# tmaklin/kbo

Measured on AMD Instinct MI355X. Metric: query Mbp/sec for kbo map, k=31, 5 Mbp SBWT; bit-exact MS vs CPU, higher is better.
Workload: dtype u32

## Files before the change

kbo_amd/batch.py:

```python
import ctypes as C

import numpy as np

from . import _capi, derandomize
from ._capi import check, lib


def _prep(concat, offsets):
    concat = np.ascontiguousarray(concat, dtype=np.uint8)
    offsets = np.ascontiguousarray(offsets, dtype=np.uint64)
    return concat, offsets, len(offsets) - 1


def ms_batch(sbwt, concat, offsets, want_intervals=False):
    concat, offsets, n = _prep(concat, offsets)
    total = int(offsets[-1]) if n > 0 else 0
    d = np.zeros(max(total, 1), dtype=np.uint8)
    lo = np.zeros(max(total, 1), dtype=np.uint32) if want_intervals else None
    hi = np.zeros(max(total, 1), dtype=np.uint32) if want_intervals else None
    check(lib().kbo_ms_batch(sbwt._h, concat.ctypes.data, offsets.ctypes.data, n, d.ctypes.data,
                             lo.ctypes.data if want_intervals else None,
                             hi.ctypes.data if want_intervals else None))
    return d[:total], (lo[:total] if want_intervals else None), (hi[:total] if want_intervals else None)

# ... 398 lines not shown
            self.work = torch.zeros(self.work_bytes // 8 + 2, dtype=torch.int64, device=device)
            self.lo = torch.zeros(self.total, dtype=torch.int32, device=device) if want_intervals else None
            self.hi = torch.zeros(self.total, dtype=torch.int32, device=device) if want_intervals else None
        self.format = format
        self.want_ms = want_ms
        self.max_error_prob = max_error_prob
        self.fused = None

    def walk(self, stream=None):
        s = stream if stream is not None else self.torch.cuda.current_stream(self.device)
        check(lib().kbo_ms_batch_dev(self.sbwt._h, self.q.data_ptr(), self.off.data_ptr(), self.n_seqs,
                                     self.total, self.max_len, self.ms.data_ptr(),
                                     self.lo.data_ptr() if self.lo is not None else None,
                                     self.hi.data_ptr() if self.hi is not None else None,
                                     self.work.data_ptr(), self.work_bytes, s.cuda_stream))

    def plan_stats(self, stream=None):
        s = stream if stream is not None else self.torch.cuda.current_stream(self.device)
        out = np.zeros(20, dtype=np.uint64)
        check(lib().kbo_plan_stats_dev(self.n_seqs, self.total, self.max_len, self.k, self.work.data_ptr(), out.ctypes.data,
                                       s.cuda_stream))
        names = ("units_walked", "accepted", "failed", "levels", "entry_levels", "seed_lookups", "seed_extensions",
                 "mismatches", "units", "redo_entries", "gave_up", "guard", "tab_lookups", "tab_written", "tab_flagged",
                 "tab_unresolved", "tab_anchored", "items_noplan")
        return {n: int(v) for n, v in zip(names, out)}

    def plan_flags(self, stream=None):
        s = stream if stream is not None else self.torch.cuda.current_stream(self.device)
        out = np.zeros(self.n_seqs, dtype=np.uint8)
        check(lib().kbo_plan_flags_dev(self.n_seqs, self.total, self.max_len, self.k, self.work.data_ptr(), out.ctypes.data, s.cuda_stream))
        return out

    def long_stats(self, stream=None):
        s = stream if stream is not None else self.torch.cuda.current_stream(self.device)
        out = np.zeros(25, dtype=np.uint64)
        check(lib().kbo_long_stats_dev(self.n_seqs, self.total, self.max_len, self.k, self.work.data_ptr(), out.ctypes.data, s.cuda_stream))
        names = ("pieces", "flagged", "sub_items", "seed_lookups", "filter_lookups", "table_lookups", "second_lookups", "_",
                 "cyc_staging", "cyc_stretches", "cyc_planes", "cyc_proof", "cyc_output", "band_tried", "band_taken", "_",
                 "why_other", "why_list", "why_ext", "why_back", "why_on", "why_band_list", "why_band_ext", "why_band_back", "why_band_on")
        return {n: int(v) for n, v in zip(names, out) if n != "_"}

    def derand_translate(self, stream=None):
        s = stream if stream is not None else self.torch.cuda.current_stream(self.device)
        if self.max_len == 0 or self.max_len > 480:
            if getattr(self, "dt_work", None) is None:
                self.dt_work_bytes = int(lib().kbo_derand_work_bytes(self.n_seqs, self.total))
                self.dt_work = self.torch.zeros(self.dt_work_bytes // 8 + 2, dtype=self.torch.int64, device=self.device)
# ... 228 lines not shown
```

kbo_amd/csrc/capi_internal.hpp:

```cpp
#pragma once
#include <atomic>
#include <cstdint>
#include <map>
#include <memory>
#include <mutex>
#include <string>
#include <vector>

#include "host_util.hpp"
#include "kernels.hpp"
#include "refine.hpp"
#include "sbwt_index.hpp"

namespace kbo_host {

struct DevCopy {
    bool arena_borrowed = false;
    static bool &transient_arena_in_use()
    {
        static thread_local bool in_use = false;
        return in_use;
    }
    DevBuf arena;
    DevBuf ent;
    uint64_t n_blocks = 0;
    bool big = false;
    uint32_t pair_off = 0;
    DevBuf seed_tab;
    uint32_t seed_d = 0;
    DevBuf dtab;
    uint32_t dtab_order = 0;
    bool dtab_grouped = false;
    DevBuf anchor;
    uint32_t anchor_bits = 0;
    DevBuf fat;
    uint32_t fat_null = 0;
    DevBuf pc_text, pc_pos, pc_node;
    DevBuf dfilt;
    uint32_t dfilt_bases = 0;
    DevBuf pc_tm, seed_pos;
    DevBuf pc_t, pc_mu, pc_mc;
    bool plan_built = false;
    bool plan_failed = false;
    uint64_t bases_seen = 0;
    struct Setup {
        double layout_s = 0, cover_s = 0, lines_s = 0, seed_s = 0, dtab_s = 0, upload_s = 0;
        uint64_t rank_bytes = 0, entry_bytes = 0, pair_bytes = 0, cover_bytes = 0, lines_bytes = 0, seed_bytes = 0, dtab_bytes = 0,
                 anchor_bytes = 0;
    } setup;
    struct PlanState {
        std::atomic<int> holdoff{0};
        std::atomic<uint32_t> epoch{0};
        uint32_t *bailed = nullptr;
        std::atomic<uint32_t> bails{0};
    } plan;
    ~DevCopy()
    {
        if (plan.bailed) {
            int prev = -1;
            (void)hipGetDevice(&prev);
            if (arena.dev >= 0 && arena.dev != prev) (void)hipSetDevice(arena.dev);
            (void)hipDeviceSynchronize();
            if (arena.dev >= 0 && arena.dev != prev && prev >= 0) (void)hipSetDevice(prev);
            (void)hipHostFree(plan.bailed);
// ... 364 lines not shown
```

kbo_amd/csrc/device_batch.cpp:

```cpp
#include "../../include/kbo_hip.h"
#include "../../include/kbo_hip_tuning.h"

#include <hip/hip_runtime.h>

#include <algorithm>
#include <atomic>
#include <cstdlib>
#include <deque>
#include <memory>
#include <mutex>
#include <vector>

#include "batch_route.hpp"

using namespace kbo_host;


namespace {
struct DevWork {
    bool chunked;
    uint32_t chunk, n_slots;
    size_t scan_off, plan_off, ms_bytes, bytes;
    size_t long_off, long_bytes, derand_off, derand_bytes;
    size_t shard_off, shard_bytes;
// ... 150 lines not shown
}

int kbo_plan_stats_dev(size_t n_seqs, uint64_t total_bases, size_t max_seq_len, uint32_t k, const void *d_work,
                       uint64_t out[KBO_PLAN_STATS], void *stream)
{
    return guarded([&] {
        KBO_REQUIRE(d_work && out && n_seqs > 0 && total_bases > 0, KBO_E_BAD_ARG, "null / empty argument");
        const DevWork w = dev_work(n_seqs, total_bases, max_seq_len, k, false);
        const kbo::PlanLayout L = kbo::plan_layout(w.n_slots, total_bases);
        const uint8_t *plan = static_cast<const uint8_t *>(d_work) + w.plan_off;
        hipStream_t s = static_cast<hipStream_t>(stream);
        uint32_t ctl[16], st[kbo::kPlanStatSlots * kbo::kPlanStatWords], tot[2];
        const uint32_t last = 2u * w.n_slots;
        HIP_OK(hipMemcpyAsync(ctl, plan + L.qctl, sizeof ctl, hipMemcpyDeviceToHost, s));
        HIP_OK(hipMemcpyAsync(st, plan + L.pstats, sizeof st, hipMemcpyDeviceToHost, s));
        HIP_OK(hipMemcpyAsync(&tot[0], plan + L.ucount + (size_t)last * 4, 4, hipMemcpyDeviceToHost, s));
        HIP_OK(hipMemcpyAsync(&tot[1], plan + L.usums + (size_t)(last / 1024u) * 4, 4, hipMemcpyDeviceToHost, s));
        HIP_OK(hipStreamSynchronize(s));
        for (uint32_t i = 0; i < KBO_PLAN_STATS; i++) out[i] = 0;
        for (uint32_t sl = 0; sl < kbo::kPlanStatSlots; sl++) {
            for (uint32_t i = 0; i < 8; i++) out[i] += st[sl * kbo::kPlanStatWords + i];
            for (uint32_t i = 0; i < 3; i++) out[12 + i] += st[sl * kbo::kPlanStatWords + kbo::kPlanStatTabLookups + i];
            out[16] += st[sl * kbo::kPlanStatWords + kbo::kPlanStatTabAnchored];
        }
        out[15] = ctl[4];
        out[17] = ctl[5];
        out[8] = (uint64_t)tot[0] + tot[1];
        out[9] = ctl[1];
        out[10] = ctl[2];
        out[11] = ctl[3];
    });
}

int kbo_plan_flags_dev(size_t n_seqs, uint64_t total_bases, size_t max_seq_len, uint32_t k, const void *d_work, uint8_t *flags_out, void *stream)
{
    return guarded([&] {
        KBO_REQUIRE(d_work && flags_out && n_seqs > 0 && total_bases > 0, KBO_E_BAD_ARG, "null / empty argument");
        const DevWork w = dev_work(n_seqs, total_bases, max_seq_len, k, false);
        KBO_REQUIRE(!w.chunked, KBO_E_UNSUPPORTED, "one item per sequence only (reads)");
        const kbo::PlanLayout L = kbo::plan_layout(w.n_slots, total_bases);
        hipStream_t s = static_cast<hipStream_t>(stream);
        HIP_OK(hipMemcpyAsync(flags_out, static_cast<const uint8_t *>(d_work) + w.plan_off + L.redo, n_seqs, hipMemcpyDeviceToHost, s));
        HIP_OK(hipStreamSynchronize(s));
    });
}

// ... 840 lines not shown
```

kbo_amd/csrc/device_index.cpp:

```cpp
#include "capi_internal.hpp"
#include "map_text.hpp"

#include <cmath>

#include <atomic>
#include <chrono>
#include <cstdlib>

namespace kbo_host {

std::atomic<int> g_waves_per_cu{0};
std::atomic<bool> g_force_big{false};
std::atomic<uint64_t> g_pair_min_rows{24ull << 20};
std::atomic<bool> g_plan_enabled{true};
std::atomic<int> g_plan_cap_div{1};
std::atomic<int> g_seed_table_depth{0};
std::atomic<int> g_depth_table{0};
std::atomic<int> g_depth_table_anchors{-1};

bool plan_enabled(const kbo_index *idx)
{
    const int v = idx ? idx->opts.plan.load() : kOptInherit;
    return v == kOptInherit ? g_plan_enabled.load() : v != 0;
}
// ... 234 lines not shown
        dc->setup.dtab_bytes = kbo::dtab_bytes((uint32_t)order, grouped) + (dc->dfilt_bases ? ((uint64_t)1 << (2u * dc->dfilt_bases)) / 8u : 0u);
        dc->setup.anchor_bytes = dc->anchor_bits ? ((uint64_t)1 << dc->anchor_bits) * 8 : 0;
    }
    dc->setup.seed_bytes = dc->seed_d ? (uint64_t)8 << (2u * dc->seed_d) : 0;
    if (dc->dtab_order >= 4 && dc->seed_d >= 4) {
        t0 = clk::now();
        const uint64_t units = kbo::pack_text_units(idx->host.n_sets);
        dc->pc_tm.alloc(units * 8 + 64);
        const uint64_t mu_bytes = kbo::pack_text_mu_bytes(units);
        dc->pc_t.alloc(units * 4 + 64);
        dc->pc_mu.alloc(mu_bytes + 64);
        dc->pc_mc.alloc(kbo::maptext::kCells / 8u);
        HIP_OK(hipMemsetAsync(dc->pc_t.as<uint8_t>() + units * 4, 0, 64, bs));
        HIP_OK(hipMemsetAsync(dc->pc_mu.as<uint8_t>() + mu_bytes, 0xFF, 64, bs));
        HIP_OK(kbo::launch_pack_text(dc->pc_text.as<uint8_t>(), pc.text.size(), dc->pc_tm.as<uint2>(), dc->pc_t.as<uint32_t>(), dc->pc_mu.as<uint32_t>(), dc->pc_mc.as<uint32_t>(), units,
                                     bs));
        dc->seed_pos.alloc(((size_t)4 << (2u * dc->seed_d)) + 64);
        HIP_OK(kbo::launch_seed_pos(dc->seed_tab.as<uint2>(), dc->pc_pos.as<uint32_t>(), dc->seed_pos.as<uint32_t>(), dc->seed_d, bs));
        HIP_OK(hipStreamSynchronize(bs));
        dc->setup.cover_bytes += units * 12 + mu_bytes + kbo::maptext::kCells / 8u;
        dc->setup.seed_bytes += (uint64_t)4 << (2u * dc->seed_d);
        idx->plan_bytes += units * 12 + mu_bytes + kbo::maptext::kCells / 8u + ((size_t)4 << (2u * dc->seed_d));
        dc->setup.seed_s += since(t0);
    }
    dc->plan_built = true;
}

uint64_t plan_break_even_bases(const kbo_index *idx)
{
    const int64_t set = g_plan_lazy_bases.load();
    if (set >= 0) return (uint64_t)set;
    const double rows = (double)idx->host.n_sets;
    const double setup_s = rows * ((idx->cover ? 0.0 : 50e-9) + 15e-9);
    if (setup_s < 0.1) return 0;
    return (uint64_t)(setup_s / 7e-12);
}
}

namespace {
void layout_from_device_rows(const kbo_index *idx, const uint64_t *d_rows, const uint8_t *d_lcs, size_t n_words, uint64_t n_blocks,
                             uint4 *d_rank, uint8_t *d_ent, uint4 *d_pair)
{
    const uint64_t n_rows = idx->host.n_sets;
    DevBuf d_scr(kbo::device_layout_scratch_bytes(n_rows));
    const uint64_t *rows_dev[4];
    for (int c = 0; c < 4; c++) rows_dev[c] = d_rows + (size_t)c * n_words;
// ... 73 lines not shown
            dc->setup.rank_bytes = rank_bytes;
            dc->setup.entry_bytes = ent_bytes;
            dc->setup.pair_bytes = pair_bytes;
            dc->setup.upload_s = since(t0);
        } catch (...) {
            delete dc;
            if (prev != device) (void)hipSetDevice(prev);
            throw;
        }
        if (prev != device) HIP_OK(hipSetDevice(prev));
        it = idx->dev.emplace(device, dc).first;
    }
    DevCopy *dc = it->second;
    const bool plan_on = plan_enabled(idx);
    if (prepare && dc->plan_failed && !dc->plan_built) dc->plan_failed = false;
    if (!dc->plan_built && !dc->plan_failed && plan_on && !idx->transient) {
        dc->bases_seen += work_bases;
        if (prepare || dc->bases_seen >= plan_break_even_bases(idx)) {
            int prev = current_device();
            if (prev != device) HIP_OK(hipSetDevice(device));
            try {
                build_plan_structures(idx, dc);
            } catch (const KboError &e) {
                for (DevBuf *b : {&dc->pc_text, &dc->pc_pos, &dc->pc_node, &dc->fat, &dc->seed_tab, &dc->dtab, &dc->anchor, &dc->dfilt, &dc->pc_tm, &dc->pc_t, &dc->pc_mu, &dc->pc_mc, &dc->seed_pos})
                    b->release();
                dc->seed_d = dc->dtab_order = dc->anchor_bits = dc->dfilt_bases = 0;
                dc->dtab_grouped = false;
                dc->fat_null = 0;
                dc->plan_failed = true;
                (void)hipGetLastError();
                if (prev != device) (void)hipSetDevice(prev);
                if (prepare) throw;
                last_error() = std::string("plan structures not built (the copy walks plainly): ") + e.what();
            } catch (...) {
                if (prev != device) (void)hipSetDevice(prev);
                throw;
            }
            if (prev != device && !dc->plan_failed) HIP_OK(hipSetDevice(prev));
        }
    }
    if (plan) *plan = &dc->plan;
    kbo::DevIndexView v;
    v.arena = dc->arena.as<uint4>();
    v.n_blocks = (uint32_t)dc->n_blocks;
    v.lcs_off = (uint32_t)(dc->n_blocks * 4 + 1);
    v.pair_off = dc->pair_off;
    v.ent = dc->big ? dc->ent.as<uint8_t>() : nullptr;
    v.big = dc->big ? 1u : 0u;
    v.n = (uint32_t)idx->host.n_sets;
    v.k = idx->host.k;
    v.pc_text = (plan_on && dc->pc_text.p) ? dc->pc_text.as<uint8_t>() + kbo::kPlanPad : nullptr;
    v.pc_pos = dc->pc_pos.as<uint32_t>();
    v.seed_tab = dc->seed_d ? dc->seed_tab.as<uint2>() : nullptr;
    v.seed_d = dc->seed_d;
    const bool use_tab = dc->dtab_order != 0 && depth_table_setting(idx) >= 0;
    v.dtab = use_tab ? dc->dtab.as<uint8_t>() : nullptr;
    v.dtab_order = use_tab ? dc->dtab_order : 0u;
    v.dtab_grouped = dc->dtab_grouped ? 1u : 0u;
    v.anchor = (use_tab && dc->anchor_bits) ? dc->anchor.as<uint64_t>() : nullptr;
    v.anchor_bits = dc->anchor_bits;
    v.fat = dc->fat.p ? dc->fat.as<uint8_t>() : nullptr;
    v.fat_null = dc->fat_null;
    v.pc_node = dc->pc_node.as<uint32_t>();
    v.pc_tm = (use_tab && dc->pc_tm.p) ? dc->pc_tm.as<uint2>() : nullptr;
    v.pc_t = (v.pc_tm && dc->pc_t.p && dc->pc_mu.p && dc->pc_mc.p) ? dc->pc_t.as<uint32_t>() : nullptr;
    v.pc_mu = v.pc_t ? dc->pc_mu.as<uint8_t>() : nullptr;
    v.pc_mc = v.pc_t ? dc->pc_mc.as<uint32_t>() : nullptr;
    v.pc_mc_shift = kbo::maptext::cell_shift(kbo::pack_text_units(idx->host.n_sets));
    v.dfilt = (use_tab && dc->dfilt_bases) ? dc->dfilt.as<uint32_t>() : nullptr;
    v.dfilt_bases = v.dfilt ? dc->dfilt_bases : 0u;
    v.seed_pos = (use_tab && dc->seed_pos.p) ? dc->seed_pos.as<uint32_t>() : nullptr;
    for (int c = 0; c < 4; c++) v.C[c] = (uint32_t)idx->host.C[c];
    v.C[4] = v.n;
    return v;
}

namespace {
constexpr int kPlanHoldoff = 16;
std::atomic<uint32_t> g_plan_epoch{1};
}

void plan_reset_holdoff() { g_plan_epoch.fetch_add(1); }

void plan_after_launch(const kbo::WalkArgs &a, hipStream_t stream, DevCopy::PlanState *ps)
{
    if (!a.gitems || !a.qctl || !ps || !ps->bailed) return;
    (void)hipMemcpyAsync(ps->bailed, a.qctl + 2, 8, hipMemcpyDeviceToHost, stream);
}

void attach_plan(kbo::WalkArgs &a, void *plan_work, DevCopy::PlanState *ps)
{
    a.gitems = nullptr;
    a.glist = nullptr;
// ... 53 lines not shown
```

kbo_amd/csrc/kernels.hpp:

```cpp
#pragma once
#include <hip/hip_runtime.h>

#include <cstdint>

#include "refset_plan.hpp"

namespace kbo {

struct DevIndexView {
    const uint4 *arena;
    uint32_t n_blocks;
    uint32_t lcs_off;
    uint32_t pair_off;
    const uint8_t *ent;
    uint32_t big;
    uint32_t n;
    uint32_t k;
    const uint8_t *pc_text;
    const uint32_t *pc_pos;
    const uint32_t *pc_node;
    uint32_t C[5];
    const uint2 *seed_tab;
    uint32_t seed_d;
    const uint8_t *fat;
    uint32_t fat_null;
    const uint8_t *dtab;
    uint32_t dtab_order;
    uint32_t dtab_grouped;
    const uint64_t *anchor;
    uint32_t anchor_bits;
    const uint2 *pc_tm;
    const uint32_t *seed_pos;
    const uint32_t *pc_t;
    const uint8_t *pc_mu;
    const uint32_t *pc_mc;
    uint32_t pc_mc_shift;
    const uint32_t *dfilt;
    uint32_t dfilt_bases;
};

struct alignas(16) WalkItem {
    uint64_t start;
    uint32_t len;
    uint32_t warm;
};

constexpr uint32_t kPlanPad = 64;
constexpr uint32_t kPlanList = 12;
constexpr uint32_t kPlanListMax = 28;
constexpr uint32_t kPlanNone = 0xFF;
constexpr uint32_t kPlanInf = 0xFFFE;
struct alignas(16) GuidedItem {
    uint32_t start;
    uint32_t p0;
    uint16_t len;
    uint16_t j_conv;
    uint16_t mm0;
    uint8_t warm;
    uint8_t n_mm;
};
enum : uint32_t { kUnitHead = 1u, kUnitPlain = 2u, kUnitToEnd = 4u };
// ... 46 lines not shown
    uint32_t *call_counts;
    uint32_t call_cap;
    uint32_t call_thr;
    uint32_t table_mode;
    uint32_t table_fused;
    uint32_t redo_piece;
    uint32_t max_item_len;
    const uint32_t *n_items_dev;
    uint8_t *chars_out;
    uint32_t map_thr, map_fmt, map_want_ms;
    uint32_t *host_bailed;
    uint32_t *run_counts;
    const uint64_t *seq_off;
    uint32_t uniform_len;
    const uint32_t *qp;
    uint32_t qp_wps;
    const uint32_t *qp_data, *qp_sums;
    const uint8_t *qp_exc;
    uint32_t *packed_out;
    uint4 *summary_out;
};
enum : uint32_t { kPlanStatUnits = 0, kPlanStatAccepted, kPlanStatFailed, kPlanStatLevels, kPlanStatEntryLevels,
                  kPlanStatSeedLookups, kPlanStatSeedExtensions, kPlanStatMismatches,
                  kPlanStatTabLookups, kPlanStatTabWritten, kPlanStatTabFlagged, kPlanStatTabAnchored, kPlanStatWords };
constexpr uint32_t kPlanStatSlots = 8;
struct PlanLayout {
    size_t gitems, units, glist, ucount, usums, qctl, pstats, redo, end;
    uint32_t unit_cap;
};
inline size_t plan_unit_cap(size_t n_items, uint64_t total_bases) { return 3 * n_items + total_bases / 64 + 64; }
inline PlanLayout plan_layout(size_t n_items, uint64_t total_bases)
{
    PlanLayout L;
    size_t w = 0;
    L.gitems = w;
    w += n_items * sizeof(GuidedItem);
    L.unit_cap = (uint32_t)(plan_unit_cap(n_items, total_bases) < 0x7FFFFF00ull ? plan_unit_cap(n_items, total_bases) : 0x7FFFFF00ull);
    L.units = w;
    w += (size_t)L.unit_cap * sizeof(WalkUnit);
    L.glist = w;
    w += (n_items * kPlanListMax * 2 + 15) / 16 * 16;
    L.ucount = w;
    w += (2 * n_items + 1) * 4;
    L.usums = w;
    w += (n_items / 512 + 4) * 4;
    w = (w + 15) / 16 * 16;
    L.qctl = w;
    w += 64;
    L.pstats = w;
    w += kPlanStatSlots * kPlanStatWords * 4;
    L.redo = w;
    w += (n_items + 15) / 16 * 16;
    L.end = w;
    return L;
}
inline size_t plan_work_bytes(size_t n_items, uint64_t total_bases) { return plan_layout(n_items, total_bases).end + 64; }
hipError_t launch_plan(WalkArgs &a, hipStream_t stream);
hipError_t launch_ms_walk_guided(WalkArgs a, uint32_t grid, uint32_t threads, hipStream_t stream);
hipError_t launch_plan_table(WalkArgs &a, hipStream_t stream);
hipError_t launch_dtab_resolve(const WalkArgs &a, hipStream_t stream);
hipError_t launch_pack_text(const uint8_t *d_text_padded, uint64_t n_bytes, uint2 *d_out, uint32_t *d_t, uint32_t *d_mu, uint32_t *d_mc, uint64_t n_units,
                            hipStream_t stream);
constexpr uint32_t kMapPad = 192;
inline uint64_t pack_text_units(uint64_t n_sets) { return (n_sets + kMapPad + 256u) / 16u + 2u; }
inline uint64_t pack_text_mu_bytes(uint64_t n_units) { return (n_units + 255u) / 256u * 32u; }
hipError_t launch_seed_pos(const uint2 *d_seed_tab, const uint32_t *d_pc_pos, uint32_t *d_out, uint32_t seed_d, hipStream_t stream);
bool map_reads_applies(const WalkArgs &a);
hipError_t launch_map_reads(WalkArgs &a, hipStream_t stream);
bool map_reads_finish_applies(const WalkArgs &a);
hipError_t launch_map_reads_finish(const WalkArgs &a, hipStream_t stream, bool one_wave_groups = false);
bool map_reads_direct(const WalkArgs &a);
bool map_reads_summary_applies(const DevIndexView &ix, uint32_t longest);
bool map_reads_packed_applies(const WalkArgs &a, bool packed_out);
hipError_t launch_flag_exceptions(const uint64_t *d_pos, uint32_t n, uint64_t base, const uint64_t *d_off, uint32_t n_seqs, uint8_t *d_exc, hipStream_t stream);
hipError_t launch_unpack_flagged(const uint32_t *d_packed, const uint64_t *d_off, uint32_t n_seqs, uint32_t uniform_wps, const uint32_t *d_scratch,
                                 const uint8_t *d_flags, uint8_t *d_q, hipStream_t stream);
hipError_t launch_pack_flagged(const uint8_t *d_chars, const uint64_t *d_off, uint32_t n_seqs, uint32_t uniform_wps, const uint32_t *d_scratch,
                               const uint8_t *d_flags, uint32_t *d_packed, hipStream_t stream);
hipError_t launch_redo_pass(WalkArgs a, hipStream_t stream);
hipError_t launch_derand_flagged(const uint8_t *d_ms, const uint64_t *d_offsets, uint32_t n_seqs, uint32_t k, uint32_t threshold,
                                 const uint8_t *d_ref, uint8_t *d_chars_out, const uint8_t *d_flags, uint32_t max_seq_len, hipStream_t stream,
                                 uint32_t *d_run_counts = nullptr);
constexpr uint32_t kDtabStretchCap = 96, kDtabStretchBlockBytes = 16u + kDtabStretchCap * 16u;
hipError_t launch_dtab_stretches(const WalkArgs &a, uint32_t n_waves, hipStream_t stream);
size_t dtab_tmp_bytes(uint64_t frontier_cap);
inline size_t dtab_bytes(uint32_t order, bool grouped) { return grouped ? (size_t)64 << (2u * (order - 2u)) : (size_t)1 << (2u * order); }
hipError_t regroup_depth_table(const uint8_t *d_plain, uint32_t order, uint8_t *d_grouped, hipStream_t stream);
hipError_t build_depth_table(const DevIndexView &ix, uint32_t order, uint8_t *d_tab, void *d_tmp, uint64_t frontier_cap, hipStream_t stream,
// ... 399 lines not shown
```

kbo_amd/csrc/map_kernels.hip:

```cpp
#include "device_util.hpp"
#include "map_text.hpp"

#include <algorithm>
#include <atomic>
#include <cstdlib>
#include <type_traits>

#ifndef KBO_STAGE_UNROLL
#define KBO_STAGE_UNROLL 6
#endif
#ifndef KBO_MAP_LB
#define KBO_MAP_LB 256
#endif
namespace kbo {
extern std::atomic<int> g_plan_cap;
namespace {

__device__ __forceinline__ void st_range16(uint8_t *o, const uint4 &v, uint32_t lo, uint32_t hi)
{
#pragma unroll
    for (uint32_t t = 0; t < 16; t++) {
        const uint32_t w = (t >> 2) == 0 ? v.x : (t >> 2) == 1 ? v.y : (t >> 2) == 2 ? v.z : v.w;
        if (t >= lo && t < hi) o[t] = (uint8_t)(w >> ((t & 3u) * 8u));
    }
// ... 56 lines not shown
        d[0] = v.x;
        d[1] = v.y;
        d[2] = v.z;
        d[3] = v.w;
    }
    __device__ __forceinline__ uint32_t word(uint64_t u) const { return p[u]; }
};
struct TextMarkBits {
    const uint8_t *p;
    __device__ __forceinline__ uint32_t from(uint64_t u) const
    {
        uint32_t w;
        __builtin_memcpy(&w, p + (u >> 3), 4);
        return w >> (uint32_t)(u & 7u);
    }
};
struct TextUnits {
    const uint2 *p;
    __device__ __forceinline__ uint32_t marks(uint64_t u) const { return p[u].y; }
};
struct WaveAny {
    __device__ __forceinline__ bool operator()(bool b) const { return __ballot(b) != 0; }
};

__global__ __launch_bounds__(64) void mark_cells_kernel(const uint8_t *__restrict__ mu, uint32_t *__restrict__ out, uint32_t shift, uint64_t n_units)
{
    const uint32_t c = blockIdx.x * 64u + threadIdx.x;
    const uint64_t any = __ballot(maptext::cell_marked(TextMarkBits{mu}, c, shift, n_units));
    if (threadIdx.x == 0u) {
        out[c >> 5] = (uint32_t)any;
        out[(c >> 5) + 1u] = (uint32_t)(any >> 32);
    }
}

__device__ __forceinline__ bool thr_gt(uint32_t thr, uint32_t order) { return thr > order; }
constexpr uint32_t kMapWords = 10;
static_assert(kMapWords == maptext::kWords, "map_text.hpp's window is a read's");
#ifdef KBO_MAP_EXPERIMENTS
constexpr bool kMapExp = true;
#else
constexpr bool kMapExp = false;
#endif
constexpr uint32_t kMapSlack = 48;
constexpr uint32_t kMapPend = 20, kMapPendBytes = kMapPend * 8u + 16u;
__host__ __device__ __forceinline__ uint32_t map_char_bytes(bool direct, uint32_t stage_bytes) { return direct ? ((stage_bytes >> 2) + 15u) & ~15u : stage_bytes; }
__host__ __device__ __forceinline__ uint32_t map_wave_lds(bool direct, uint32_t stage_bytes, uint32_t lin_words)
// ... 218 lines not shown
                }
                e += (kMapExp && (a.rounds & 4u)) ? (D + 1u) / 2u : D;
            }
        }
    }
    if (plannable && !has_invalid && !seeded && have_amb) {
        seeded = true;
        p0 = p_amb;
    }

    const TextDigits text_d{a.ix.pc_t};
    const TextMarkBits text_mu{a.ix.pc_mu};
    const TextUnits text_tm{a.ix.pc_tm};
    auto near_mark = [&](uint32_t q) -> bool {
        const uint32_t c = maptext::cell_of(q >> 4, a.ix.pc_mc_shift);
        return (__shfl(mark_cells, (int)((c >> 5) & 63u)) >> (c & 31u)) & 1u;
    };
    auto compare = [&](uint32_t pd, bool near, uint32_t (&mm)[kMapWords]) -> uint32_t {
        return maptext::compare_split(text_d, text_mu, text_tm, WaveAny{}, near, qw, pd + kMapPad, len, mm);
    };
    uint32_t cnt = 0;
    uint32_t junction = 0xFFu;
    uint32_t jov = 0;
    uint32_t mmw[kMapWords];
#pragma unroll
    for (uint32_t g = 0; g < kMapWords; g++) mmw[g] = 0;
    if (__ballot(seeded)) {
        const bool nm = near_mark(p0 + kMapPad);
        if (seeded) cnt = compare(p0, nm, mmw);
    }
    if (DIRECT) {
        const uint32_t listmax = a.plan_list + 1u;
        uint32_t tail_c = 0;
#pragma unroll
        for (uint32_t g = 0; g < kMapWords; g++) {
            const uint32_t lo_b = 16u * g, t0 = len - 16u;
            if (lo_b + 16u > t0 && lo_b < len) tail_c += (uint32_t)__popc(mmw[g] & (t0 > lo_b ? (1u << (2u * (16u - (t0 - lo_b)))) - 1u : ~0u));
        }
        const bool dense = seeded && len >= 32u && (tail_c >= 6u || (uint32_t)__popc(mmw[0]) >= 6u) && !(kMapExp && (a.rounds & 8u));
        const bool need2 = plannable && !has_invalid && len >= 2u * D && (!seeded || cnt > listmax || dense);
        if (__ballot(need2)) {
            uint32_t pB = 0, eb = len - 1u, tries = 0;
            bool seedB = false;
            const uint32_t lowest = len > cap ? len - cap : 0u;
            const bool near = need2 && seeded && 10u * cnt <= 7u * len && !(kMapExp && (a.rounds & 8u));
            bool front = false;
// ... 72 lines not shown
                        b0 = w == w0 ? mmB[w] : b0;
                        b1 = w == w0 + 1u ? mmB[w] : b1;
                        if (w < w0) c0 = c0 + (uint32_t)__popc(mmw[w]) - (uint32_t)__popc(mmB[w]);
                    }
                    uint32_t gcut = 16u * w0, cmin = c0, cc = c0;
                    for (uint32_t x = 0; x < 32u; x++) {
                        const uint32_t wa = x < 16u ? a0 : a1, wb = x < 16u ? b0 : b1, sh = 2u * (15u - (x & 15u));
                        cc = cc + ((wa >> sh) & 1u) - ((wb >> sh) & 1u);
                        if (16u * w0 + x + 1u <= len && cc <= cmin) {
                            cmin = cc;
                            gcut = 16u * w0 + x + 1u;
                        }
                    }
                    if (cB <= cmin) gcut = 0u;
                    if (gcut == 0u) {
#pragma unroll
                        for (uint32_t g = 0; g < kMapWords; g++) mmw[g] = mmB[g];
                        cnt = cB;
                        p0 = pB;
                    } else if (gcut < len) {
                        uint32_t jm = 0xFFu, before = 0;
                        int32_t lastA = -1;
                        cnt = 0;
#pragma unroll
                        for (uint32_t g = 0; g < kMapWords; g++) {
                            const uint32_t lo_b = 16u * g;
                            uint32_t keepA = gcut <= lo_b ? 0u : (gcut >= lo_b + 16u ? ~0u : ~0u << (32u - 2u * (gcut - lo_b)));
                            if (mmw[g] & keepA) lastA = (int32_t)(lo_b + 15u - ((uint32_t)__builtin_ctz(mmw[g] & keepA) >> 1));
                            uint32_t m1 = (mmw[g] & keepA) | (mmB[g] & ~keepA);
                            if (gcut - 1u >= lo_b && gcut - 1u < lo_b + 16u) {
                                const uint32_t bit = 0x40000000u >> (2u * (gcut - 1u - lo_b));
                                if (!(m1 & bit)) {
                                    jm = before + (uint32_t)__popc(m1 & ~(bit | (bit - 1u)));
                                    m1 |= bit;
                                }
                            }
                            before += (uint32_t)__popc(m1);
                            mmw[g] = m1;
                            cnt += (uint32_t)__popc(m1);
                        }
                        junction = jm;
                        if (jm != 0xFFu) {
                            const uint32_t E = gcut - 1u, W = E >> 4;
                            uint32_t wlo = 0, whi = 0;
#pragma unroll
                            for (uint32_t g = 0; g < kMapWords; g++) {
// ... 33 lines not shown
    }
    if (DIRECT && seeded && cnt > a.plan_list + 1u && 3u * cnt > len && !(a.rounds & 64u)) {
        seeded = false;
        junction = 0xFFu;
        jov = 0;
        cnt = 0;
    }
    bool flag = plannable && seeded && cnt > a.plan_list + 1u;
    const bool no_plan = plannable && !seeded && !has_invalid;
    flag = flag || (plannable && has_invalid);
    if (!DIRECT) {
        const uint32_t first_mm = (seeded && cnt > 0) ? (uint32_t)sp[0] : len;
        const uint32_t lim = (seeded && !flag) ? min(min(k - 1u, first_mm), len) : 0u;
        const uint32_t most = min(k - 1u, 16u * kMapWords);
        for (uint32_t i = 0; i < most; i++) {
            if (__ballot(i < lim) == 0) break;
            if (i < lim) so[soff + i] = (uint8_t)(i + 1u);
        }
    }

    bool w_around = false, w_unsettled = false;
    uint32_t w_e = 0, w_owner = 0, w_at = 0, w_len = 0, w_pre[6] = {0, 0, 0, 0, 0, 0};
    uint32_t st_look = 0, st_written = 0, st_anch = 0, st_filt = 0;
    {
        const uint32_t order = a.ix.dtab_order;
        const bool have_anch = DIRECT && a.ix.anchor != nullptr && thr_gt(a.map_thr, order);
        const uint32_t thr = a.map_thr, covb = DIRECT ? thr - order + 2u : 1u, cov = have_anch ? thr - order : covb;
        const uint32_t n_blockwin = (DIRECT && len > thr) ? (len - order + covb - 1u) / covb + 1u : 0u;
        const uint32_t my_n = !plannable || flag ? 0u : DIRECT ? (no_plan ? (n_blockwin + 3u) / 4u : (len > thr ? cnt : 0u))
                                                               : (no_plan ? (len + 15u) / 16u : cnt);
        uint32_t incl = my_n;
#pragma unroll
        for (int off = 1; off < 64; off <<= 1) {
            const uint32_t t = __shfl_up(incl, off);
            if ((int)lane >= off) incl += t;
        }
        const uint32_t total = __shfl(incl, 63);
        sp[13] = 0;
        if (lane == 0) *pend_n = 0;
        *reinterpret_cast<uint16_t *>(sp + 14) = (uint16_t)incl;
        __builtin_amdgcn_fence(__ATOMIC_ACQ_REL, "wavefront");
        __builtin_amdgcn_wave_barrier();
        using code_t = typename std::conditional<NP == 16, uint32_t, uint64_t>::type;
        const code_t omask = (code_t)((1ull << (2u * order)) - 1ull);
        for (uint32_t w0 = 0; w0 < total; w0 += 64u) {
            const uint32_t w = w0 + lane;
            const bool work = w < total;
            uint32_t lo_l = 0, hi_l = 63;
#pragma unroll
            for (int it = 0; it < 6; it++) {
                const uint32_t mid = (lo_l + hi_l) >> 1;
                const uint32_t pm = *reinterpret_cast<const uint16_t *>(spw + mid * 16u + 14u);
                if (pm > w) hi_l = mid;
                else lo_l = mid + 1u;
            }
            const uint32_t owner = work ? lo_l : lane;
            const uint32_t o_incl = __shfl(incl, (int)owner), o_n = __shfl(my_n, (int)owner), o_soff = __shfl(soff, (int)owner),
                           o_len = __shfl(len, (int)owner), o_np = __shfl(no_plan ? 1u : 0u, (int)owner), o_junc = __shfl(junction, (int)owner), o_jov = __shfl(jov, (int)owner);
            const bool blockmode = o_np != 0;
            if (DIRECT) {
                if (work) {
                    const uint32_t t = w - (o_incl - o_n);
                    const uint32_t m = blockmode ? 0u : (uint32_t)spw[owner * 16u + t];
                    uint32_t bytes[4], ee[4];
                    bool use[4], lastw[4], look[4];
#pragma unroll
                    for (uint32_t i = 0; i < 4u; i++) {
                        if (blockmode) {
                            const uint32_t u = 4u * t + i;
                            ee[i] = min(order - 1u + u * covb, o_len - 1u);
                            use[i] = o_len >= order && (u == 0u || order - 1u + (u - 1u) * covb < o_len - 1u);
                            lastw[i] = true;
                        } else {
                            const uint32_t jn = t == o_junc ? 1u + o_jov : 0u, j1 = t == o_junc ? 1u : 0u;
                            ee[i] = m + j1 + min(i * cov, order - 1u - jn);
                            use[i] = ee[i] < o_len && ee[i] + 1u >= order && (i == 0u || (i - 1u) * cov < order - 1u - jn);
                            lastw[i] = i * cov >= order - 1u - jn;
                        }
                        bytes[i] = 0;
                        look[i] = use[i];
                    }
                    if (a.ix.dfilt) {
                        const uint32_t F = a.ix.dfilt_bases, fmask = (1u << (2u * F)) - 1u;
                        uint32_t zlo, zhi;
                        if (blockmode) zlo = zhi = 0xFFFFFFFFu;
                        else if (t == o_junc) { zlo = m - o_jov; zhi = m + 1u; }
                        else zlo = zhi = m;
                        if (blockmode || zhi - zlo < F) {
                            uint32_t fw[4][2];
                            bool two[4];
#pragma unroll
                            for (uint32_t i = 0; i < 4u; i++) {
                                fw[i][0] = fw[i][1] = 0xFFFFFFFFu;
                                two[i] = false;
                                if (use[i]) {
                                    const uint32_t e = ee[i], left = e - (order - F);
                                    const uint32_t e1 = blockmode ? e : min(e, zlo + F - 1u), e2 = blockmode ? left : max(zhi, left);
                                    const uint32_t k1 = (uint32_t)ending_at(o_soff + e1) & fmask, k2 = (uint32_t)ending_at(o_soff + e2) & fmask;
                                    fw[i][0] = a.ix.dfilt[k1 >> 5] >> (k1 & 31u);
                                    two[i] = kMapExp && e2 != e1 && (a.rounds & 2u);
                                    if (two[i]) fw[i][1] = a.ix.dfilt[k2 >> 5] >> (k2 & 31u);
                                    if (STATS) st_filt += two[i] ? 2u : 1u;
                                }
                            }
#pragma unroll
// ... 416 lines not shown
                r_ = iv.y;
                alive = l_ < r_;
            }
            const uint8_t *arena_ = reinterpret_cast<const uint8_t *>(a.ix.arena);
            for (uint32_t j_ = D_; j_ <= thr; j_++) {
                if (__ballot(alive) == 0) break;
                if (alive) {
                    const uint32_t cb_ = base_at(first + j_) * a.ix.n_blocks, bl_ = div96(l_), br_ = div96(r_);
                    const uint4 xA = ld16(arena_, (cb_ + bl_) << 4), xB = ld16(arena_, (cb_ + br_) << 4);
                    l_ = rank_eval(xA, l_ - bl_ * 96u);
                    r_ = rank_eval(xB, r_ - br_ * 96u);
                    alive = l_ < r_;
                }
            }
            if (__ballot(alive) != 0 && lane == 0) spw[own_ * 16u + 13u] = 1;
        }
        __builtin_amdgcn_fence(__ATOMIC_ACQ_REL, "wavefront");
        __builtin_amdgcn_wave_barrier();
        flag = flag || sp[13] != 0;
    }
    if (STATS) plan_stats_add(a.pstats, kPlanStatSeedLookups, st_lookups, kPlanStatSeedExtensions, st_filt , kPlanStatMismatches, seeded ? cnt : 0u, 0, 0);
    if (STATS) plan_stats_add(a.pstats, kPlanStatTabLookups, st_look, kPlanStatTabWritten, st_written, kPlanStatTabFlagged, flag ? 1u : 0u,
                   kPlanStatTabAnchored, st_anch);
    const uint64_t fm = __ballot(flag), nm = __ballot(no_plan);
    if (lane == 0) {
        if (fm) atomicAdd(a.qctl + 4, (uint32_t)__popcll(fm));
        if (nm) atomicAdd(a.qctl + 5, (uint32_t)__popcll(nm));
    }
    if (have_item) a.redo[idx] = flag ? 1 : 0;
    if (SUM && have_item && !flag) a.summary_out[idx] = summary;
    if (flag && have_item) reinterpret_cast<uint32_t *>(a.units)[atomicAdd(a.qctl + 6, 1u)] = idx;
}

constexpr uint32_t kFinishStride = 176, kFinishMaxR = 16, kFinishWaves = 8192, kFinishLds = 2u * kFinishMaxR * kFinishStride;
template <bool SUM = false>
__global__ __launch_bounds__(256) void finish_reads_kernel(WalkArgs a, uint32_t r1, uint32_t r4)
{
    extern __shared__ __attribute__((aligned(16))) uint8_t fin_lds_all[];
    const uint32_t lane = threadIdx.x & 63u;
    uint8_t *lds = fin_lds_all + (threadIdx.x >> 6) * kFinishLds;
    const uint32_t wave = blockIdx.x * (blockDim.x >> 6) + (threadIdx.x >> 6), n_waves = gridDim.x * (blockDim.x >> 6);
    const uint32_t n_f = min(a.qctl[6], a.n_items);
    if (wave == 0 && lane == 0 && a.qctl[4] > a.unit_bail) {
        a.qctl[2] = 1;
        if (a.host_bailed) *a.host_bailed = 1u;
    }
// ... 91 lines not shown
            if (len >= 3u)
                for (uint32_t p = s; p < len; p += L) {
                    uint32_t ch = mL[p];
                    if (a.map_fmt) ch = (ch == 'M' || ch == 'R') ? (uint32_t)qL[p] : (uint32_t)'-';
                    a.chars_out[o0 + p] = (uint8_t)ch;
                }
        }
        __builtin_amdgcn_fence(__ATOMIC_ACQ_REL, "wavefront");
        __builtin_amdgcn_wave_barrier();
    }
}

}

hipError_t launch_pack_text(const uint8_t *d_text_padded, uint64_t n_bytes, uint2 *d_out, uint32_t *d_t, uint32_t *d_mu, uint32_t *d_mc, uint64_t n_units,
                            hipStream_t stream)
{
    hipLaunchKernelGGL(pack_text_kernel, dim3((unsigned)((n_units + 255) / 256)), dim3(256), 0, stream, d_text_padded, n_bytes, d_out, d_t, d_mu, n_units);
    hipLaunchKernelGGL(mark_cells_kernel, dim3(maptext::kCells / 64u), dim3(64), 0, stream, reinterpret_cast<const uint8_t *>(d_mu), d_mc,
                       maptext::cell_shift(n_units), n_units);
    return hipGetLastError();
}

hipError_t launch_seed_pos(const uint2 *d_seed_tab, const uint32_t *d_pc_pos, uint32_t *d_out, uint32_t seed_d, hipStream_t stream)
{
    const uint64_t n = 1ull << (2u * seed_d);
    hipLaunchKernelGGL(seed_pos_kernel, dim3((unsigned)((n + 255) / 256)), dim3(256), 0, stream, d_seed_tab, d_pc_pos, d_out, n);
    return hipGetLastError();
}

static bool map_reads_index_applies(const DevIndexView &ix, uint32_t longest)
{
    return ix.dtab && ix.pc_tm && ix.pc_t && ix.pc_mu && ix.pc_mc && ix.seed_pos && ix.seed_d >= 4u && ix.seed_d <= 14u && ix.dtab_order >= 4u && ix.dtab_order <= 17u &&
           ix.dtab_order <= ix.k && longest != 0 && longest <= 16u * kMapWords;
}
bool map_reads_applies(const WalkArgs &a)
{
    return map_reads_index_applies(a.ix, a.max_item_len) && !a.call_sites && !a.lo_out && a.redo && a.qctl && a.units;
}

bool map_reads_direct(const WalkArgs &a)
{
    static const int env_direct = std::getenv("KBO_MAP_DIRECT") ? std::atoi(std::getenv("KBO_MAP_DIRECT")) : 1;
    const uint32_t sp_w = (a.ix.anchor && a.map_thr > a.ix.dtab_order) ? a.map_thr - a.ix.dtab_order : a.map_thr - a.ix.dtab_order + 2u;
    return env_direct != 0 && !a.map_want_ms && a.ix.dtab_order <= a.map_thr && a.map_thr < a.ix.k && (a.ix.dtab_order - 1u + sp_w - 1u) / sp_w + 1u <= 4u;
}

bool map_reads_packed_applies(const WalkArgs &a, bool packed_out) { (void)packed_out; return map_reads_applies(a) && map_reads_direct(a) && !a.map_fmt; }

hipError_t launch_map_reads(WalkArgs &a, hipStream_t stream)
{
    if (a.n_items == 0) return hipSuccess;
    a.table_mode = 1;
    a.table_fused = 1;
    a.unit_bail = a.n_items / 2u + 64u;
    a.plan_list = kPlanList;
    a.plan_cap = (uint32_t)g_plan_cap.load();
    static const int env_x = std::getenv("KBO_MAP_X") ? std::atoi(std::getenv("KBO_MAP_X")) : 0;
    a.rounds = (uint32_t)env_x;
    a.redo_piece = 16u;
    hipError_t e = hipMemsetAsync(a.qctl, 0, 64 + kPlanStatSlots * kPlanStatWords * 4, stream);
    if (e != hipSuccess) return e;
    const bool direct = map_reads_direct(a);
    static const bool env_nouni = std::getenv("KBO_MAP_NO_UNIFORM") != nullptr;
    a.uniform_len = (a.seq_off && !env_nouni && a.max_item_len != 0 && (uint64_t)a.n_items * a.max_item_len == a.q_bytes) ? a.max_item_len : 0u;
    const int io = a.qp ? (a.packed_out ? 2 : 1) : 0;
    if (io != 0 && (!direct || a.map_fmt)) return hipErrorInvalidValue;
    const uint32_t stage_bytes = io ? (64u * 16u * ((a.max_item_len + 15u) / 16u) + 32u + kMapSlack) : (64u * a.max_item_len + 16u + kMapSlack + 15u) / 16u * 16u;
    const uint32_t lin_words = stage_bytes / 16u + 4u;
    const uint32_t lds_wave = map_wave_lds(direct, stage_bytes, lin_words);
    static const int env_wpb = std::getenv("KBO_MAP_WPB") ? std::atoi(std::getenv("KBO_MAP_WPB")) : 1;
    const uint32_t wpb = (uint32_t)std::min(4, std::max(1, env_wpb));
    const uint32_t n_waves = (a.n_items + 63u) / 64u;
    const dim3 grid((n_waves + wpb - 1u) / wpb), block(64u * wpb);
    static const int env_pad = std::getenv("KBO_MAP_LDS_PAD") ? std::atoi(std::getenv("KBO_MAP_LDS_PAD")) : 0;
    const uint32_t lds = lds_wave * wpb + (uint32_t)env_pad;
#define KBO_MAP_LAUNCH(NP_, DIRECT_, IO_)                                                                                                         \
    do {                                                                                                                                          \
        if (a.pstats) hipLaunchKernelGGL((map_reads_kernel<NP_, DIRECT_, IO_, true>), grid, block, lds, stream, a, stage_bytes, lin_words);       \
        else hipLaunchKernelGGL((map_reads_kernel<NP_, DIRECT_, IO_, false>), grid, block, lds, stream, a, stage_bytes, lin_words);               \
    } while (0)
#define KBO_MAP_LAUNCH_SUM(NP_, DIRECT_, IO_) \
    hipLaunchKernelGGL((map_reads_kernel<NP_, DIRECT_, IO_, false, true>), grid, block, lds, stream, a, stage_bytes, lin_words)
    if (a.summary_out) {
        if (io == 2 || a.pstats || a.chars_out || a.d_out || a.run_counts || a.map_fmt || a.map_want_ms) return hipErrorInvalidValue;
        if (a.ix.dtab_order <= 15u) {
// ... 54 lines not shown
```

Before: 1.146 million.

## Precompute per-position substitution-clean bitmap to skip table lookups for isolated mismatches

At index build time, a new kernel marks every text position where substituting any other base yields no dtab hit across all windows, and stores the result as a bitmap. In the map_reads kernel, an isolated mismatch (not a junction or cut, with neighbours at least order apart) consults this bit; if it is set, the per-window dtab lookups and the dfilt check are skipped. This removes random table accesses on the common single-substitution path. The cost is extra index memory, a setup kernel, and added branching. The bitmap is only used when the threshold and anchor configuration match those it was built with.

```diff
diff --git a/kbo_amd/batch.py b/kbo_amd/batch.py
--- a/kbo_amd/batch.py
+++ b/kbo_amd/batch.py
@@ -444,7 +444,7 @@
                                        s.cuda_stream))
         names = ("units_walked", "accepted", "failed", "levels", "entry_levels", "seed_lookups", "seed_extensions",
                  "mismatches", "units", "redo_entries", "gave_up", "guard", "tab_lookups", "tab_written", "tab_flagged",
-                 "tab_unresolved", "tab_anchored", "items_noplan")
+                 "tab_unresolved", "tab_anchored", "items_noplan", "subst_bits", "subst_clean")
         return {n: int(v) for n, v in zip(names, out)}
 
     def plan_flags(self, stream=None):
diff --git a/kbo_amd/csrc/capi_internal.hpp b/kbo_amd/csrc/capi_internal.hpp
--- a/kbo_amd/csrc/capi_internal.hpp
+++ b/kbo_amd/csrc/capi_internal.hpp
@@ -40,6 +40,9 @@
     uint32_t dfilt_bases = 0;
     DevBuf pc_tm, seed_pos;
     DevBuf pc_t, pc_mu, pc_mc;
+    DevBuf sub_clean;
+    uint32_t sub_thr = 0;
+    bool sub_anch = false;
     bool plan_built = false;
     bool plan_failed = false;
     uint64_t bases_seen = 0;
diff --git a/kbo_amd/csrc/device_batch.cpp b/kbo_amd/csrc/device_batch.cpp
--- a/kbo_amd/csrc/device_batch.cpp
+++ b/kbo_amd/csrc/device_batch.cpp
@@ -196,6 +196,8 @@
             for (uint32_t i = 0; i < 8; i++) out[i] += st[sl * kbo::kPlanStatWords + i];
             for (uint32_t i = 0; i < 3; i++) out[12 + i] += st[sl * kbo::kPlanStatWords + kbo::kPlanStatTabLookups + i];
             out[16] += st[sl * kbo::kPlanStatWords + kbo::kPlanStatTabAnchored];
+            out[18] += st[sl * kbo::kPlanStatWords + kbo::kPlanStatSubstBits];
+            out[19] += st[sl * kbo::kPlanStatWords + kbo::kPlanStatSubstClean];
         }
         out[15] = ctl[4];
         out[17] = ctl[5];
diff --git a/kbo_amd/csrc/device_index.cpp b/kbo_amd/csrc/device_index.cpp
--- a/kbo_amd/csrc/device_index.cpp
+++ b/kbo_amd/csrc/device_index.cpp
@@ -1,4 +1,5 @@
 #include "capi_internal.hpp"
+#include "map_subst.hpp"
 #include "map_text.hpp"
 
 #include <cmath>
@@ -280,6 +281,30 @@
         dc->setup.seed_bytes += (uint64_t)4 << (2u * dc->seed_d);
         idx->plan_bytes += units * 12 + mu_bytes + kbo::maptext::kCells / 8u + ((size_t)4 << (2u * dc->seed_d));
         dc->setup.seed_s += since(t0);
+        const char *env_sub = std::getenv("KBO_SUBST_BITS");
+        kbo_map_opts dflt;
+        kbo_map_opts_default(&dflt);
+        const size_t thr = idx->host.n_kmers > 0 ? random_match_threshold(idx->host.k, idx->host.n_kmers, 4, dflt.max_error_prob) : 0;
+        const bool anch = dc->anchor_bits != 0 && thr > dc->dtab_order;
+        const uint32_t step = thr >= dc->dtab_order ? kbo::mapsubst::window_step(dc->dtab_order, (uint32_t)thr, anch) : 0u;
+        if (!(env_sub && std::atoi(env_sub) == 0) && thr >= dc->dtab_order && thr < idx->host.k && !kbo::mapsubst::window_used(kbo::mapsubst::kWindows, step, dc->dtab_order, 0u)) {
+            t0 = clk::now();
+            const uint64_t sub_bytes = kbo::mapsubst::bitmap_words(units) * 4;
+            dc->sub_clean.alloc(sub_bytes + 64);
+            HIP_OK(hipMemsetAsync(dc->sub_clean.as<uint8_t>() + sub_bytes, 0, 64, bs));
+            kbo::DevIndexView sv{};
+            sv.pc_tm = dc->pc_tm.as<uint2>();
+            sv.dtab = dc->dtab.as<uint8_t>();
+            sv.dtab_order = dc->dtab_order;
+            sv.dtab_grouped = dc->dtab_grouped ? 1u : 0u;
+            HIP_OK(kbo::launch_subst_bits(sv, units, (uint32_t)thr, anch, dc->sub_clean.as<uint32_t>(), bs));
+            HIP_OK(hipStreamSynchronize(bs));
+            dc->sub_thr = (uint32_t)thr;
+            dc->sub_anch = anch;
+            dc->setup.cover_bytes += sub_bytes;
+            idx->plan_bytes += sub_bytes;
+            dc->setup.cover_s += since(t0);
+        }
     }
     dc->plan_built = true;
 }
@@ -399,7 +424,7 @@
             try {
                 build_plan_structures(idx, dc);
             } catch (const KboError &e) {
-                for (DevBuf *b : {&dc->pc_text, &dc->pc_pos, &dc->pc_node, &dc->fat, &dc->seed_tab, &dc->dtab, &dc->anchor, &dc->dfilt, &dc->pc_tm, &dc->pc_t, &dc->pc_mu, &dc->pc_mc, &dc->seed_pos})
+                for (DevBuf *b : {&dc->pc_text, &dc->pc_pos, &dc->pc_node, &dc->fat, &dc->seed_tab, &dc->dtab, &dc->anchor, &dc->dfilt, &dc->pc_tm, &dc->pc_t, &dc->pc_mu, &dc->pc_mc, &dc->sub_clean, &dc->seed_pos})
                     b->release();
                 dc->seed_d = dc->dtab_order = dc->anchor_bits = dc->dfilt_bases = 0;
                 dc->dtab_grouped = false;
@@ -446,6 +471,9 @@
     v.pc_mc_shift = kbo::maptext::cell_shift(kbo::pack_text_units(idx->host.n_sets));
     v.dfilt = (use_tab && dc->dfilt_bases) ? dc->dfilt.as<uint32_t>() : nullptr;
     v.dfilt_bases = v.dfilt ? dc->dfilt_bases : 0u;
+    v.sub_clean = (v.pc_t && dc->sub_clean.p) ? dc->sub_clean.as<uint32_t>() : nullptr;
+    v.sub_thr = dc->sub_thr;
+    v.sub_anch = dc->sub_anch ? 1u : 0u;
     v.seed_pos = (use_tab && dc->seed_pos.p) ? dc->seed_pos.as<uint32_t>() : nullptr;
     for (int c = 0; c < 4; c++) v.C[c] = (uint32_t)idx->host.C[c];
     v.C[4] = v.n;
diff --git a/kbo_amd/csrc/kernels.hpp b/kbo_amd/csrc/kernels.hpp
--- a/kbo_amd/csrc/kernels.hpp
+++ b/kbo_amd/csrc/kernels.hpp
@@ -37,6 +37,8 @@
     uint32_t pc_mc_shift;
     const uint32_t *dfilt;
     uint32_t dfilt_bases;
+    const uint32_t *sub_clean;
+    uint32_t sub_thr, sub_anch;
 };
 
 struct alignas(16) WalkItem {
@@ -129,7 +131,9 @@
 };
 enum : uint32_t { kPlanStatUnits = 0, kPlanStatAccepted, kPlanStatFailed, kPlanStatLevels, kPlanStatEntryLevels,
                   kPlanStatSeedLookups, kPlanStatSeedExtensions, kPlanStatMismatches,
-                  kPlanStatTabLookups, kPlanStatTabWritten, kPlanStatTabFlagged, kPlanStatTabAnchored, kPlanStatWords };
+                  kPlanStatTabLookups, kPlanStatTabWritten, kPlanStatTabFlagged, kPlanStatTabAnchored,
+                  kPlanStatSubstBits, kPlanStatSubstClean,
+                  kPlanStatWords };
 constexpr uint32_t kPlanStatSlots = 8;
 struct PlanLayout {
     size_t gitems, units, glist, ucount, usums, qctl, pstats, redo, end;
@@ -171,6 +175,7 @@
 constexpr uint32_t kMapPad = 192;
 inline uint64_t pack_text_units(uint64_t n_sets) { return (n_sets + kMapPad + 256u) / 16u + 2u; }
 inline uint64_t pack_text_mu_bytes(uint64_t n_units) { return (n_units + 255u) / 256u * 32u; }
+hipError_t launch_subst_bits(const DevIndexView &ix, uint64_t n_units, uint32_t thr, bool have_anch, uint32_t *d_bits, hipStream_t stream);
 hipError_t launch_seed_pos(const uint2 *d_seed_tab, const uint32_t *d_pc_pos, uint32_t *d_out, uint32_t seed_d, hipStream_t stream);
 bool map_reads_applies(const WalkArgs &a);
 hipError_t launch_map_reads(WalkArgs &a, hipStream_t stream);
diff --git a/kbo_amd/csrc/map_kernels.hip b/kbo_amd/csrc/map_kernels.hip
--- a/kbo_amd/csrc/map_kernels.hip
+++ b/kbo_amd/csrc/map_kernels.hip
@@ -1,4 +1,5 @@
 #include "device_util.hpp"
+#include "map_subst.hpp"
 #include "map_text.hpp"
 
 #include <algorithm>
@@ -102,6 +103,38 @@
 struct WaveAny {
     __device__ __forceinline__ bool operator()(bool b) const { return __ballot(b) != 0; }
 };
+
+static_assert(mapsubst::kPad == kMapPad, "map_subst.hpp keys its bits by the 2-bit text's positions");
+struct SubstBits {
+    const uint32_t *p;
+    __device__ __forceinline__ uint32_t word(uint64_t w) const { return p[w]; }
+};
+struct SubstText {
+    const uint2 *tm;
+    uint64_t n_units;
+    __device__ __forceinline__ uint64_t positions() const { return 16ull * n_units; }
+    __device__ __forceinline__ bool marked(uint64_t q) const { return (tm[q >> 4].y >> (2u * (15u - (uint32_t)(q & 15u)))) & 1u; }
+    __device__ __forceinline__ uint32_t base(uint64_t q) const { return (tm[q >> 4].x >> (2u * (15u - (uint32_t)(q & 15u)))) & 3u; }
+};
+struct SubstTable {
+    const uint8_t *dtab;
+    uint32_t order, grouped;
+    __device__ __forceinline__ bool present(uint64_t key) const
+    {
+        return (dtab[grouped ? dtab_grouped_addr(key, 0u, order) : key] & 0x80u) != 0u;
+    }
+};
+__global__ __launch_bounds__(256) void subst_bits_kernel(SubstText tx, SubstTable tab, uint32_t thr, uint32_t have_anch, uint32_t *__restrict__ out,
+                                                         uint64_t n_words)
+{
+    const uint64_t q = (uint64_t)blockIdx.x * blockDim.x + threadIdx.x;
+    const bool c = q < tx.positions() && mapsubst::clean(tx, tab, q, tab.order, thr, have_anch != 0u);
+    const uint64_t any = __ballot(c);
+    if ((threadIdx.x & 63u) == 0u) {
+        if ((q >> 5) < n_words) out[q >> 5] = (uint32_t)any;
+        if ((q >> 5) + 1u < n_words) out[(q >> 5) + 1u] = (uint32_t)(any >> 32);
+    }
+}
 
 __global__ __launch_bounds__(64) void mark_cells_kernel(const uint8_t *__restrict__ mu, uint32_t *__restrict__ out, uint32_t shift, uint64_t n_units)
 {
@@ -366,6 +399,7 @@
     uint32_t cnt = 0;
     uint32_t junction = 0xFFu;
     uint32_t jov = 0;
+    bool cut = false;
     uint32_t mmw[kMapWords];
 #pragma unroll
     for (uint32_t g = 0; g < kMapWords; g++) mmw[g] = 0;
@@ -484,6 +518,7 @@
                         uint32_t jm = 0xFFu, before = 0;
                         int32_t lastA = -1;
                         cnt = 0;
+                        cut = true;
 #pragma unroll
                         for (uint32_t g = 0; g < kMapWords; g++) {
                             const uint32_t lo_b = 16u * g;
@@ -563,10 +598,11 @@
     bool w_around = false, w_unsettled = false;
     uint32_t w_e = 0, w_owner = 0, w_at = 0, w_len = 0, w_pre[6] = {0, 0, 0, 0, 0, 0};
     uint32_t st_look = 0, st_written = 0, st_anch = 0, st_filt = 0;
+    uint32_t st_bits = 0, st_clean = 0;
     {
         const uint32_t order = a.ix.dtab_order;
         const bool have_anch = DIRECT && a.ix.anchor != nullptr && thr_gt(a.map_thr, order);
-        const uint32_t thr = a.map_thr, covb = DIRECT ? thr - order + 2u : 1u, cov = have_anch ? thr - order : covb;
+        const uint32_t thr = a.map_thr, covb = DIRECT ? mapsubst::window_step(order, thr, false) : 1u, cov = DIRECT ? mapsubst::window_step(order, thr, have_anch) : 1u;
         const uint32_t n_blockwin = (DIRECT && len > thr) ? (len - order + covb - 1u) / covb + 1u : 0u;
         const uint32_t my_n = !plannable || flag ? 0u : DIRECT ? (no_plan ? (n_blockwin + 3u) / 4u : (len > thr ? cnt : 0u))
                                                                : (no_plan ? (len + 15u) / 16u : cnt);
@@ -598,6 +634,7 @@
             const uint32_t owner = work ? lo_l : lane;
             const uint32_t o_incl = __shfl(incl, (int)owner), o_n = __shfl(my_n, (int)owner), o_soff = __shfl(soff, (int)owner),
                            o_len = __shfl(len, (int)owner), o_np = __shfl(no_plan ? 1u : 0u, (int)owner), o_junc = __shfl(junction, (int)owner), o_jov = __shfl(jov, (int)owner);
+            const uint32_t o_p0 = __shfl(p0, (int)owner), o_cut = __shfl(cut ? 1u : 0u, (int)owner);
             const bool blockmode = o_np != 0;
             if (DIRECT) {
                 if (work) {
@@ -605,6 +642,18 @@
                     const uint32_t m = blockmode ? 0u : (uint32_t)spw[owner * 16u + t];
                     uint32_t bytes[4], ee[4];
                     bool use[4], lastw[4], look[4];
+                    bool lone = false, settled = false;
+                    if (a.ix.sub_clean && !blockmode) {
+                        const uint8_t *osp = spw + owner * 16u;
+                        const bool has_prev = t > 0u, has_next = t + 1u < o_n;
+                        lone = mapsubst::eligible(false, o_cut != 0u, t == o_junc, has_prev, has_prev ? (uint32_t)osp[t - 1u] : 0u, m, has_next,
+                                                  has_next ? (uint32_t)osp[t + 1u] : 0u, order);
+                        if (lone) {
+                            settled = mapsubst::clean_bit(SubstBits{a.ix.sub_clean}, mapsubst::bit_of(o_p0, m));
+                            if (STATS) st_bits++;
+                            if (STATS && settled) st_clean++;
+                        }
+                    }
 #pragma unroll
                     for (uint32_t i = 0; i < 4u; i++) {
                         if (blockmode) {
@@ -614,14 +663,14 @@
                             lastw[i] = true;
                         } else {
                             const uint32_t jn = t == o_junc ? 1u + o_jov : 0u, j1 = t == o_junc ? 1u : 0u;
-                            ee[i] = m + j1 + min(i * cov, order - 1u - jn);
-                            use[i] = ee[i] < o_len && ee[i] + 1u >= order && (i == 0u || (i - 1u) * cov < order - 1u - jn);
-                            lastw[i] = i * cov >= order - 1u - jn;
+                            ee[i] = m + j1 + mapsubst::window_offset(i, cov, order, jn);
+                            use[i] = ee[i] < o_len && ee[i] + 1u >= order && mapsubst::window_used(i, cov, order, jn);
+                            lastw[i] = mapsubst::window_last(i, cov, order, jn);
                         }
                         bytes[i] = 0;
-                        look[i] = use[i];
-                    }
-                    if (a.ix.dfilt) {
+                        look[i] = use[i] && !settled;
+                    }
+                    if (a.ix.dfilt && !lone) {
                         const uint32_t F = a.ix.dfilt_bases, fmask = (1u << (2u * F)) - 1u;
                         uint32_t zlo, zhi;
                         if (blockmode) zlo = zhi = 0xFFFFFFFFu;
@@ -1084,6 +1133,7 @@
     if (STATS) plan_stats_add(a.pstats, kPlanStatSeedLookups, st_lookups, kPlanStatSeedExtensions, st_filt , kPlanStatMismatches, seeded ? cnt : 0u, 0, 0);
     if (STATS) plan_stats_add(a.pstats, kPlanStatTabLookups, st_look, kPlanStatTabWritten, st_written, kPlanStatTabFlagged, flag ? 1u : 0u,
                    kPlanStatTabAnchored, st_anch);
+    if (STATS) plan_stats_add(a.pstats, kPlanStatSubstBits, st_bits, kPlanStatSubstClean, st_clean, 0, 0, 0, 0);
     const uint64_t fm = __ballot(flag), nm = __ballot(no_plan);
     if (lane == 0) {
         if (fm) atomicAdd(a.qctl + 4, (uint32_t)__popcll(fm));
@@ -1221,6 +1271,14 @@
     return hipGetLastError();
 }
 
+hipError_t launch_subst_bits(const DevIndexView &ix, uint64_t n_units, uint32_t thr, bool have_anch, uint32_t *d_bits, hipStream_t stream)
+{
+    const uint64_t n_words = mapsubst::bitmap_words(n_units);
+    hipLaunchKernelGGL(subst_bits_kernel, dim3((unsigned)((32u * n_words + 255u) / 256u)), dim3(256), 0, stream, SubstText{ix.pc_tm, n_units},
+                       SubstTable{ix.dtab, ix.dtab_order, ix.dtab_grouped}, thr, have_anch ? 1u : 0u, d_bits, n_words);
+    return hipGetLastError();
+}
+
 hipError_t launch_seed_pos(const uint2 *d_seed_tab, const uint32_t *d_pc_pos, uint32_t *d_out, uint32_t seed_d, hipStream_t stream)
 {
     const uint64_t n = 1ull << (2u * seed_d);
@@ -1261,6 +1319,7 @@
     hipError_t e = hipMemsetAsync(a.qctl, 0, 64 + kPlanStatSlots * kPlanStatWords * 4, stream);
     if (e != hipSuccess) return e;
     const bool direct = map_reads_direct(a);
+    if (!direct || a.map_thr != a.ix.sub_thr || (a.ix.sub_anch != 0u) != (a.ix.anchor != nullptr && a.map_thr > a.ix.dtab_order)) a.ix.sub_clean = nullptr;
     static const bool env_nouni = std::getenv("KBO_MAP_NO_UNIFORM") != nullptr;
     a.uniform_len = (a.seq_off && !env_nouni && a.max_item_len != 0 && (uint64_t)a.n_items * a.max_item_len == a.q_bytes) ? a.max_item_len : 0u;
     const int io = a.qp ? (a.packed_out ? 2 : 1) : 0;
diff --git a/kbo_amd/csrc/map_subst.hpp b/kbo_amd/csrc/map_subst.hpp
--- /dev/null
+++ b/kbo_amd/csrc/map_subst.hpp
@@ -0,0 +1,52 @@
+#pragma once
+#include <stdint.h>
+
+#if defined(__HIPCC__) || defined(__HIP__)
+#define KBO_MS_FN __host__ __device__ __forceinline__
+#else
+#define KBO_MS_FN inline
+#endif
+
+namespace kbo {
+namespace mapsubst {
+
+constexpr uint32_t kWindows = 4;
+constexpr uint32_t kPad = 192;
+
+KBO_MS_FN uint32_t window_step(uint32_t order, uint32_t thr, bool have_anch) { return have_anch ? thr - order : thr - order + 2u; }
+KBO_MS_FN uint32_t window_offset(uint32_t i, uint32_t cov, uint32_t order, uint32_t jn) { return i * cov < order - 1u - jn ? i * cov : order - 1u - jn; }
+KBO_MS_FN bool window_used(uint32_t i, uint32_t cov, uint32_t order, uint32_t jn) { return i == 0u || (i - 1u) * cov < order - 1u - jn; }
+KBO_MS_FN bool window_last(uint32_t i, uint32_t cov, uint32_t order, uint32_t jn) { return i * cov >= order - 1u - jn; }
+
+KBO_MS_FN bool eligible(bool block_mode, bool cut, bool junction, bool has_prev, uint32_t prev, uint32_t m, bool has_next, uint32_t next, uint32_t order)
+{
+    return !block_mode && !cut && !junction && (!has_prev || m - prev > order - 1u) && (!has_next || next - m > order - 1u);
+}
+
+KBO_MS_FN uint64_t bit_of(uint32_t p0, uint32_t m) { return (uint64_t)(uint32_t)(p0 + m + kPad); }
+KBO_MS_FN uint64_t bitmap_words(uint64_t n_units) { return (n_units + 1u) / 2u; }
+template <class Bits> KBO_MS_FN bool clean_bit(const Bits &bits, uint64_t q) { return (bits.word(q >> 5) >> (uint32_t)(q & 31u)) & 1u; }
+
+template <class Text, class Table>
+KBO_MS_FN bool clean(const Text &tx, const Table &tab, uint64_t q, uint32_t order, uint32_t thr, bool have_anch, uint32_t leave_out = 0u)
+{
+    if (order < 2u || order > 32u || thr < order || (have_anch && thr == order)) return false;
+    if (q + 1u < order || q + order > tx.positions()) return false;
+    for (uint64_t x = q + 1u - order; x < q + order; x++)
+        if (tx.marked(x)) return false;
+    const uint32_t cov = window_step(order, thr, have_anch), own = tx.base(q);
+    for (uint32_t i = 0; i < kWindows; i++) {
+        if (!window_used(i, cov, order, 0u) || ((leave_out >> i) & 1u)) continue;
+        const uint32_t o = window_offset(i, cov, order, 0u);
+        uint64_t key = 0;
+        for (uint32_t j = 0; j < order; j++) key = (key << 2) | tx.base(q + o + 1u - order + j);
+        for (uint32_t b = 0; b < 4u; b++) {
+            if (b == own) continue;
+            if (tab.present((key & ~(3ull << (2u * o))) | ((uint64_t)b << (2u * o)))) return false;
+        }
+    }
+    return !window_used(kWindows, cov, order, 0u);
+}
+
+}
+}
```

Result: faster. 1.291 million, median of 6 (+12.6%).
